# tanhuajie/Pytorch-RT1-for-Distributed-Training

Measured on AMD Instinct MI355X. Metric: train samples/sec (whole node), RT-1 Language-Table, 1/2/4/8 MI355X, higher is better.
Workload: dtype bf16; 1 GPU; model=RT-1 (FiLM-EfficientNet-B3 + TokenLearner-8 + 8-layer transformer, 35.3M params), global_batch=128, batch_per_gpu=128, seq_len=6, parallelism=dp1, backend=hip, hipgraph=True, step=graph, graph_segments=1, tuned_library_gemms=True, full=False

## Files before the change

pytorch_rt1_for_distributed_training_amd/csrc/bindings.cpp:

```cpp
#include <algorithm>
#include <cmath>
#include <cstdlib>

#include <torch/extension.h>
#include <c10/hip/HIPStream.h>
#include <hip/hip_runtime.h>

#include "rt1_kernels.h"

namespace {

hipStream_t cur_stream() { return c10::hip::getCurrentHIPStream().stream(); }

bool sync_check() {
    static const bool on = [] {
        const char* e = std::getenv("RT1_SYNC_CHECK");
        return e != nullptr && *e != '\0' && *e != '0';
    }();
    return on;
}

void check_launch(int err, const char* what) {
    TORCH_CHECK(err == 0, what, ": HIP launch failed: ", hipGetErrorString((hipError_t)err));
    if (sync_check()) {
// ... 777 lines not shown
    } else {
        check_launch(rt1_dw_bwd_fused(bp(dA), y2p, gate.data_ptr<float>(), rb.data_ptr<float>(), sc2.data_ptr<float>(),
                                      sh2.data_ptr<float>(), mu2.data_ptr<float>(), rs2.data_ptr<float>(),
                                      g2.data_ptr<float>(), mdz2.data_ptr<float>(), mdzx2.data_ptr<float>(),
                                      w.data_ptr<float>(), nullptr, nullptr, sc1.data_ptr<float>(), sh1.data_ptr<float>(),
                                      1, mu1.data_ptr<float>(), rs1.data_ptr<float>(), N, H, W, C, (int)k, gx, bp(dx),
                                      pa.data_ptr<float>(), pb.data_ptr<float>(), part.data_ptr<float>(), cur_stream(), 1,
                                      zout ? 1 : 0, bp(x), bp(we), cin),
                     "dw_bwd_fused_x");
    }
    return {dx, sum0(part).view({C, k * k}), pa, pb};
}

std::vector<at::Tensor> gemm(at::Tensor A, at::Tensor B, bool nn, OptT bias, OptT scale, OptT shift, OptT gate,
                             int64_t hw, bool out_f32, bool stats, int64_t cfg, bool store_a) {
    check_bf(A, "A"); check_bf(B, "B");
    TORCH_CHECK(A.dim() == 2 && B.dim() == 2, "gemm: 2-D operands");
    const int64_t M = A.size(0), K = A.size(1);
    const int64_t N = nn ? B.size(1) : B.size(0);
    TORCH_CHECK((nn ? B.size(0) : B.size(1)) == K, "gemm: inner dimensions differ");
    TORCH_CHECK(M > 0 && N % 8 == 0 && K % 8 == 0 && N > 0 && K > 0, "gemm: N and K must be multiples of 8");
    TORCH_CHECK(M < ((int64_t)1 << 31) && N * K < ((int64_t)1 << 31), "gemm: too large");
    TORCH_CHECK(reinterpret_cast<uintptr_t>(A.data_ptr()) % 16 == 0 && reinterpret_cast<uintptr_t>(B.data_ptr()) % 16 == 0,
                "gemm: operands must be 16-byte aligned");
    check_opt_f(bias, "bias", N);
    const bool pro = scale.has_value() && scale->defined();
    if (pro) {
        check_f(*scale, "scale", K); check_f(*shift, "shift", K);
        TORCH_CHECK(hw > 0 && M % hw == 0, "gemm: hw must divide M");
        check_f(*gate, "gate", (M / hw) * K);
        TORCH_CHECK(!out_f32, "gemm: the prologue path writes bf16");
    }
    TORCH_CHECK(!(stats && out_f32), "gemm: statistics describe a bf16 output");
    TORCH_CHECK(!store_a || pro, "gemm: store_a stores the prologue's rebuilt operand");
    auto C = at::empty({M, N}, A.options().dtype(out_f32 ? at::kFloat : at::kBFloat16));
    at::Tensor aout;
    if (store_a) aout = at::empty_like(A);
    at::Tensor ps, pq;
    if (stats) {
        const int tm = rt1_gemm_tiles_m((int)M, (int)N, (int)K, (int)cfg);
        ps = at::empty({tm, N}, f32(A));
        pq = at::empty({tm, N}, f32(A));
    }
    check_launch(rt1_gemm(bp(A), bp(B), C.data_ptr(), (int)M, (int)N, (int)K, nn ? 1 : 0, fpo(bias), fpo(scale),
                          fpo(shift), fpo(gate), (int)hw, out_f32 ? 1 : 0, stats ? ps.data_ptr<float>() : nullptr,
                          stats ? pq.data_ptr<float>() : nullptr, (int)cfg, store_a ? bp(aout) : nullptr,
                          cur_stream()), "gemm");
    std::vector<at::Tensor> out{C};
    if (stats) { out.push_back(ps); out.push_back(pq); }
    if (store_a) out.push_back(aout);
    return out;
}

at::Tensor film_fwd(at::Tensor xe, int64_t K, at::Tensor w, at::Tensor bias, at::Tensor cmap, int64_t total,
                    int64_t cfg) {
    check_bf(xe, "xe"); check_bf(w, "w");
    TORCH_CHECK(xe.dim() == 2 && w.dim() == 2 && w.size(1) == K && K <= xe.size(1), "film_fwd: xe [M, >= K], w [N, K]");
    const int64_t M = xe.size(0), N = w.size(0);
    TORCH_CHECK(M > 0 && N % 8 == 0 && K % 8 == 0 && xe.size(1) % 8 == 0, "film_fwd: N, K, lda multiples of 8");
    check_f(bias, "bias", N);
    TORCH_CHECK(cmap.is_cuda() && cmap.is_contiguous() && cmap.scalar_type() == at::kInt && cmap.numel() == N,
                "film_fwd: cmap must be an int32 [N / 4, 4] GPU tensor");
    TORCH_CHECK(total == M * N, "film_fwd: total must be M * N");
    auto out = at::empty({total}, f32(xe));
    check_launch(rt1_gemm_cmap(bp(xe), (int)xe.size(1), bp(w), out.data_ptr<float>(), (int)M, (int)N, (int)K,
                               bias.data_ptr<float>(), cmap.data_ptr<int>(), (int)cfg, cur_stream()), "film_fwd");
    return out;
}

std::vector<at::Tensor> film_wgrad(at::Tensor dflat, at::Tensor cmap, at::Tensor xe, int64_t K, int64_t splits,
                                   int64_t tile) {
    check_bf(xe, "xe");
    TORCH_CHECK(xe.dim() == 2 && K <= xe.size(1), "film_wgrad: xe [M, >= K]");
    const int64_t M = xe.size(0), N = cmap.numel();
    check_f(dflat, "dflat", M * N);
    TORCH_CHECK(cmap.is_cuda() && cmap.is_contiguous() && cmap.scalar_type() == at::kInt && N % 8 == 0 && K % 8 == 0,
                "film_wgrad: cmap int32 [N / 4, 4], N and K multiples of 8");
    auto a = xe.size(1) == K ? xe : xe.narrow(1, 0, K).contiguous();
    const int s = (int)std::max<int64_t>(1, std::min<int64_t>(splits, (M + 63) / 64));
    auto part = at::empty({s, N, K}, f32(xe));
    auto dbp = at::empty({s, N}, f32(xe));
    check_launch(rt1_wgrad_dymap(dflat.data_ptr<float>(), cmap.data_ptr<int>(), bp(a), M, (int)N, (int)K, s,
                                 part.data_ptr<float>(), dbp.data_ptr<float>(), (int)tile, cur_stream()),
                 "film_wgrad");
    if (s == 1) return {part[0], dbp[0]};
    return {sum0(part), sum0(dbp)};
}

std::vector<at::Tensor> gemm256(at::Tensor A, at::Tensor B, bool nn, OptT bias, OptT scale, OptT shift, OptT gate,
                                int64_t hw, bool stats, bool store_a, int64_t bn) {
    check_bf(A, "A"); check_bf(B, "B");
    TORCH_CHECK(A.dim() == 2 && B.dim() == 2, "gemm256: 2-D operands");
    const int64_t M = A.size(0), K = A.size(1);
    const int64_t N = nn ? B.size(1) : B.size(0);
    TORCH_CHECK((nn ? B.size(0) : B.size(1)) == K, "gemm256: inner dimensions differ");
    TORCH_CHECK(M > 0 && N > 0 && K > 0 && N % 8 == 0 && K % 8 == 0, "gemm256: N and K must be multiples of 8");
    TORCH_CHECK(M < ((int64_t)1 << 31) && M * K < ((int64_t)1 << 40), "gemm256: too large");
    TORCH_CHECK(reinterpret_cast<uintptr_t>(A.data_ptr()) % 16 == 0 && reinterpret_cast<uintptr_t>(B.data_ptr()) % 16 == 0,
                "gemm256: operands must be 16-byte aligned");
    TORCH_CHECK(bn == 128 || bn == 256, "gemm256: bn must be 128 or 256");
    check_opt_f(bias, "bias", N);
    const bool pro = scale.has_value() && scale->defined();
    if (pro) {
        TORCH_CHECK(!nn, "gemm256: the operand prologue is an NT path");
        check_f(*scale, "scale", K); check_f(*shift, "shift", K);
        TORCH_CHECK(hw > 0 && M % hw == 0, "gemm256: hw must divide M");
// ... 570 lines not shown
                           ln ? rs.data_ptr<float>() : nullptr, cur_stream()), "resid");
    if (ln) return {out, xn, mu, rs};
    return {out};
}

std::vector<at::Tensor> tf_drop_bwd(at::Tensor dout, double p, int64_t seed, OptT seed_dev) {
    check_rows512(dout, "dout", at::kFloat);
    const int T = (int)dout.size(0);
    const int grid = rt1_tf_grid(T);
    auto dh = at::empty({T, 512}, dout.options().dtype(at::kBFloat16));
    auto part = at::empty({grid, 512}, dout.options());
    check_launch(rt1_drop_bwd(dout.data_ptr<float>(), T, (float)p, (uint32_t)seed, seed_ptr(seed_dev), bp(dh),
                              part.data_ptr<float>(), grid,
                              cur_stream()), "drop_bwd");
    return {dh, sum0(part)};
}


namespace rt1comm {
void register_comm(py::module_& m);
}
namespace rt1head {
void register_head(py::module_& m);
}

PYBIND11_MODULE(_rt1_hip, m) {
    m.doc() = "RT-1 HIP/CDNA4 kernels (gfx950)";
    m.def("flat_adam", &flat_adam, "fused Adam/AdamW over flat fp32 buffers");
    m.def("flat_adam_dev", &flat_adam_dev, "fused Adam/AdamW, step/lr read from a device tensor (graph-replayable)");
    m.def("flat_adam_clip_dev", &flat_adam_clip_dev, "flat_adam_dev obeying clip_state (clip coefficient, skipped step)");
    m.def("flat_adam_ema_dev", &flat_adam_ema_dev, "flat_adam_dev / flat_adam_clip_dev that also updates the EMA of the weights");
    m.def("flat_adam_groups_dev", &flat_adam_groups_dev,
          "the device-state Adam forms (plain, clip, EMA, both) with lr / weight_decay per parameter group");
    m.def("gradnorm_partials", &gradnorm_partials, "fp64 partial sums grad_sumsq writes for n floats");
    m.def("grad_sumsq", &grad_sumsq, "deterministic sum of squares of a flat fp32 gradient -> fp64 partials");
    m.def("grad_clip_finalize", &grad_clip_finalize, "partials -> clip_state {norm, coef, ok, counters}");
    m.def("buffer_guard_", &buffer_guard_, "ok ? shadow = buf : buf = shadow");
    m.def("bn_stats", &bn_stats);
    m.def("bn_finalize", &bn_finalize);
    m.def("xgram", &xgram);
    m.def("gemm_tail", &gemm_tail, py::arg("A"), py::arg("B"), py::arg("A2"), py::arg("B2"), py::arg("bias") = py::none(),
          py::arg("res") = py::none(), py::arg("rmul") = py::none(), py::arg("rhw") = 1, py::arg("cfg") = -1);
    m.def("gemm256", &gemm256, py::arg("A"), py::arg("B"), py::arg("nn") = false, py::arg("bias") = py::none(),
          py::arg("scale") = py::none(), py::arg("shift") = py::none(), py::arg("gate") = py::none(),
          py::arg("hw") = 0, py::arg("stats") = false, py::arg("store_a") = false, py::arg("bn") = 256);
    m.def("film_fwd", &film_fwd, py::arg("xe"), py::arg("K"), py::arg("w"), py::arg("bias"), py::arg("cmap"),
          py::arg("total"), py::arg("cfg") = -1);
    m.def("film_wgrad", &film_wgrad, py::arg("dflat"), py::arg("cmap"), py::arg("xe"), py::arg("K"),
          py::arg("splits") = 1, py::arg("tile") = 0);
    m.def("gemm", &gemm, py::arg("A"), py::arg("B"), py::arg("nn") = false, py::arg("bias") = py::none(),
          py::arg("scale") = py::none(), py::arg("shift") = py::none(), py::arg("gate") = py::none(),
          py::arg("hw") = 0, py::arg("out_f32") = false, py::arg("stats") = false, py::arg("cfg") = -1,
          py::arg("store_a") = false);
    m.def("x_bn_stats", &x_bn_stats);
    m.def("bn_from_gram", &bn_from_gram);
    m.def("dw_x_supported", &dw_x_supported);
    m.def("dw_tile_info", &dw_tile_info);
    m.def("dw_fwd_x", &dw_fwd_x);
    m.def("dw_bwd_fused_x", &dw_bwd_fused_x, py::arg("dA"), py::arg("y2"), py::arg("gate"), py::arg("rb"),
          py::arg("sc2"), py::arg("sh2"), py::arg("mu2"), py::arg("rs2"), py::arg("g2"), py::arg("mdz2"),
          py::arg("mdzx2"), py::arg("w"), py::arg("k"), py::arg("x"), py::arg("we"), py::arg("sc1"), py::arg("sh1"),
          py::arg("mu1"), py::arg("rs1"), py::arg("max_blocks"), py::arg("zout") = true);
    m.def("bn_apply", &bn_apply);
    m.def("bn_bwd_reduce", &bn_bwd_reduce);
    m.def("bn_bwd_finalize", &bn_bwd_finalize);
    m.def("bn_bwd_finalize_new", &bn_bwd_finalize_new);
    m.def("bn_bwd_finalize_pw", &bn_bwd_finalize_pw);
    m.def("bn_bwd_apply", &bn_bwd_apply, py::arg("G"), py::arg("rs"), py::arg("rb"), py::arg("HW"), py::arg("y"),
          py::arg("scale"), py::arg("shift"), py::arg("mean"), py::arg("rstd"), py::arg("gamma"), py::arg("act"),
          py::arg("mdz"), py::arg("mdzx"), py::arg("keep") = py::none());
    m.def("dw_fwd", &dw_fwd);
    m.def("dw_bwd_data", &dw_bwd_data);
    m.def("dw_bwd_weight", &dw_bwd_weight);
    m.def("dw_bwd_fused", &dw_bwd_fused, py::arg("dA"), py::arg("y2"), py::arg("gate"), py::arg("rb"), py::arg("sc2"),
          py::arg("sh2"), py::arg("mu2"), py::arg("rs2"), py::arg("g2"), py::arg("mdz2"), py::arg("mdzx2"), py::arg("w"),
          py::arg("k"), py::arg("x1"), py::arg("sc1"), py::arg("sh1"), py::arg("act1"), py::arg("mu1"), py::arg("rs1"),
          py::arg("max_blocks"), py::arg("variant") = -1, py::arg("zout") = false, py::arg("res") = py::none(),
          py::arg("rmul") = py::none());
    m.def("gram", &gram, "{x^T x, sum_m x} fp32 of x [M, C] bf16 in one MFMA pass", py::arg("x"),
          py::arg("variant") = -1, py::arg("splits") = 0);
    m.def("wgrad", &wgrad, "1x1-conv weight gradient dy^T a on MFMA (optional BN/act/gate prologue on a)",
          py::arg("dy"), py::arg("a"), py::arg("scale") = py::none(), py::arg("shift") = py::none(),
          py::arg("gate") = py::none(), py::arg("act") = 0, py::arg("hw") = 0, py::arg("variant") = -1,
          py::arg("splits") = -1, py::arg("partials") = false, py::arg("sums") = false);
    m.def("crop_resize_u8", &crop_resize_u8, "Pillow-exact random-resized-crop of raw uint8 frames (GPU)");
    m.def("crop_resize_gather_u8", &crop_resize_gather_u8,
          "crop_resize_u8 over frames gathered by index from an HBM-resident [F, h, w, 3] table");
    m.def("multi_reduce_copy_", &multi_reduce_copy_, "dst[i] = fixed-order sum of splits[i] partials of src[i]",
          py::arg("dst"), py::arg("src"), py::arg("splits"), py::arg("sstride"));
    m.def("multi_copy_", &multi_copy_, "dst[i].copy_(src[i]) for many same-dtype tensors, 128 per launch");
    m.def("multi_reduce_add_", &multi_reduce_add_, "dst[i] += fixed-order sum of splits[i] partials of src[i]",
          py::arg("dst"), py::arg("src"), py::arg("splits"), py::arg("sstride"));
    m.def("multi_add_", &multi_add_, "dst[i] += src[i] for many fp32 tensors, 128 per launch");
    m.def("colsum", &colsum_py, "deterministic fixed-order sum over dim 0 (fp32/bf16 in, fp32 out)");
    m.def("frame_pool", &frame_pool);
    m.def("block_tail", &block_tail);
    m.def("tail_bwd_reduce", &tail_bwd_reduce);
    m.def("stem_fwd", &stem_fwd);
    m.def("stem_bwd_weight", &stem_bwd_weight, py::arg("img"), py::arg("shift"), py::arg("dy"), py::arg("max_blocks"),
          py::arg("bn_x") = py::none(), py::arg("scale") = py::none(), py::arg("shift_bn") = py::none(),
          py::arg("mean") = py::none(), py::arg("rstd") = py::none(), py::arg("gamma") = py::none(),
          py::arg("mdz") = py::none(), py::arg("mdzx") = py::none());
    m.def("attn_fwd", &attn_fwd, py::arg("qkv"), py::arg("L"), py::arg("Kimg"), py::arg("scale"), py::arg("drop_p"),
          py::arg("seed"), py::arg("seed_dev") = py::none());
    m.def("se_bn_bwd_reduce", &se_bn_bwd_reduce);
    m.def("proj_bwd", &proj_bwd, "project-conv backward sums + dWp from (dy3, y2) per frame (skinny blocks)");
// ... 30 lines not shown
```

pytorch_rt1_for_distributed_training_amd/csrc/kernels/gemm.hip:

```cpp
#include "common.h"

using namespace rt1;

namespace {

typedef short bf16x8 __attribute__((ext_vector_type(8)));
typedef short bf16x4 __attribute__((ext_vector_type(4)));
typedef float f32x4 __attribute__((ext_vector_type(4)));
typedef __attribute__((address_space(3))) bf16x4 lds_v4;

constexpr int BLOCK = 256;
constexpr int BK = 64;
constexpr int LDK = BK + 8;

__device__ __forceinline__ bf16x8 tr_read8(const bf16_t* base0, const bf16_t* base1) {
    const bf16x4 a = __builtin_amdgcn_ds_read_tr16_b64_v4i16((lds_v4*)base0);
    const bf16x4 b = __builtin_amdgcn_ds_read_tr16_b64_v4i16((lds_v4*)base1);
    return bf16x8{a[0], a[1], a[2], a[3], b[0], b[1], b[2], b[3]};
}

struct GemmArgs {
    const bf16_t* A;
    const bf16_t* B;
    void* C;
// ... 251 lines not shown
                u.x = pack2(v[0], v[1]);
                u.y = pack2(v[2], v[3]);
                *reinterpret_cast<uint2*>(reinterpret_cast<bf16_t*>(g.C) + m * N + n) = u;
                if constexpr (STATS) {
                    const float s0 = __uint_as_float(u.x << 16), s1 = __uint_as_float(u.x & 0xffff0000u);
                    const float s2 = __uint_as_float(u.y << 16), s3 = __uint_as_float(u.y & 0xffff0000u);
                    ssum[i][0] += s0; ssq[i][0] = fmaf(s0, s0, ssq[i][0]);
                    ssum[i][1] += s1; ssq[i][1] = fmaf(s1, s1, ssq[i][1]);
                    ssum[i][2] += s2; ssq[i][2] = fmaf(s2, s2, ssq[i][2]);
                    ssum[i][3] += s3; ssq[i][3] = fmaf(s3, s3, ssq[i][3]);
                }
            }
        }
    }
    if constexpr (STATS) {
#pragma unroll
        for (int i = 0; i < S::NT; ++i)
#pragma unroll
            for (int e = 0; e < 4; ++e) {
#pragma unroll
                for (int o = 1; o < 16; o <<= 1) {
                    ssum[i][e] += __shfl_xor(ssum[i][e], o, 64);
                    ssq[i][e] += __shfl_xor(ssq[i][e], o, 64);
                }
            }
        __syncthreads();
        float* red = reinterpret_cast<float*>(smem);
        if (lr == 0) {
#pragma unroll
            for (int i = 0; i < S::NT; ++i)
#pragma unroll
                for (int e = 0; e < 4; ++e) {
                    const int c = wn * S::WTN + i * 16 + lh * 4 + e;
                    red[(wm * 2) * BN + c] = ssum[i][e];
                    red[(wm * 2 + 1) * BN + c] = ssq[i][e];
                }
        }
        __syncthreads();
        for (int c = t; c < BN; c += BLOCK) {
            float a = 0.f, q = 0.f;
#pragma unroll
            for (int w = 0; w < WM; ++w) {
                a += red[(w * 2) * BN + c];
                q += red[(w * 2 + 1) * BN + c];
            }
            if (n0 + c < N) {
                g.ps[(int64_t)tm * N + n0 + c] = a;
                g.pq[(int64_t)tm * N + n0 + c] = q;
            }
        }
    }
}

struct Cfg { int bm, bn; };
constexpr Cfg CFGS[] = {{128, 128}, {64, 256}, {256, 64}, {64, 64}, {128, 64}};
constexpr int NCFG = 5;

int pick_cfg(int M, int N, int K, int cfg) {
    if (cfg >= 0 && cfg < NCFG) return cfg;
    (void)K;
    if (N <= 64) return 2;
    if (M <= 16384 && N >= 1024) return 1;
    return 0;
}

template <int BM, int BN, int WM, bool NN>
int launch_cfg(const GemmArgs& a, bool pro, bool f32, bool stats, hipStream_t st) {
    using S = GShape<BM, BN, WM, NN>;
    static_assert(BM * (BN + 8) * 2 <= S::lds, "LDS-staged store tile fits");
    const int tiles = ((a.M + BM - 1) / BM) * ((a.N + BN - 1) / BN);
    const dim3 grid(tiles);
    if constexpr (!NN) {
        if (a.A2) {
            if (pro || f32 || stats) return (int)hipErrorInvalidValue;
            hipLaunchKernelGGL((gemm_kernel<BM, BN, WM, false, false, false, false, true>), grid, dim3(BLOCK), S::lds,
                               st, a);
            return (int)hipGetLastError();
        }
    } else {
        if (a.A2) return (int)hipErrorInvalidValue;
    }
    static_assert(WM * 2 * BN * 4 <= S::lds, "stats scratch fits");
#define G(P, F, ST) hipLaunchKernelGGL((gemm_kernel<BM, BN, WM, NN, P, F, ST>), grid, dim3(BLOCK), S::lds, st, a)
    if (pro) {
        if (f32) return (int)hipErrorInvalidValue;
        if (stats) G(true, false, true); else G(true, false, false);
    } else if (f32) {
        if (stats) return (int)hipErrorInvalidValue;
        G(false, true, false);
    } else {
        if (stats) G(false, false, true); else G(false, false, false);
    }
#undef G
    return (int)hipGetLastError();
}

template <bool NN>
int launch_any(int cfg, const GemmArgs& a, bool pro, bool f32, bool stats, hipStream_t st) {
    switch (cfg) {
        case 0: return launch_cfg<128, 128, 2, NN>(a, pro, f32, stats, st);
        case 1: return launch_cfg<64, 256, 1, NN>(a, pro, f32, stats, st);
        case 2: return launch_cfg<256, 64, 4, NN>(a, pro, f32, stats, st);
        case 3: return launch_cfg<64, 64, 2, NN>(a, pro, f32, stats, st);
        default: return launch_cfg<128, 64, 2, NN>(a, pro, f32, stats, st);
    }
}

}

extern "C" {

int rt1_gemm_tiles_m(int M, int N, int K, int cfg) {
    const Cfg c = CFGS[pick_cfg(M, N, K, cfg)];
    return (M + c.bm - 1) / c.bm;
}

int rt1_gemm(const bf16_t* A, const bf16_t* B, void* C, int M, int N, int K, int nn, const float* bias,
             const float* scale, const float* shift, const float* gate, int hw, int out_f32, float* ps, float* pq,
             int cfg, bf16_t* aout, hipStream_t st) {
    if (M <= 0 || N <= 0 || K <= 0 || (N % 8) || (K % 8)) return (int)hipErrorInvalidValue;
    const bool pro = scale != nullptr;
    if (pro && (!shift || !gate || hw <= 0 || M % hw)) return (int)hipErrorInvalidValue;
    if ((ps != nullptr) != (pq != nullptr) || (aout && !pro)) return (int)hipErrorInvalidValue;
    GemmArgs a{A, B, C, M, N, K, bias, scale, shift, gate, hw, ps, pq, aout, nullptr, nullptr, 0, nullptr, nullptr, 1, K,
               nullptr};
    const bool stats = ps != nullptr;
    const int c = pick_cfg(M, N, K, cfg);
    return nn ? launch_any<true>(c, a, pro, out_f32, stats, st) : launch_any<false>(c, a, pro, out_f32, stats, st);
}

int rt1_gemm_tail(const bf16_t* A, const bf16_t* B, int M, int N, int K, const bf16_t* A2, const bf16_t* B2, int K2,
                  const float* bias, const bf16_t* res, const float* rmul, int rhw, bf16_t* C, int cfg,
                  hipStream_t st) {
    if (M <= 0 || N <= 0 || K <= 0 || K2 <= 0 || (N % 8) || (K % 8) || (K2 % 8) || !A2 || !B2)
        return (int)hipErrorInvalidValue;
    if (res && (!rmul || rhw <= 0 || M % rhw)) return (int)hipErrorInvalidValue;
    GemmArgs a{A, B, C, M, N, K, bias, nullptr, nullptr, nullptr, 1, nullptr, nullptr, nullptr, A2, B2, K2, res, rmul,
               rhw > 0 ? rhw : 1, K, nullptr};
    return launch_any<false>(pick_cfg(M, N, K, cfg), a, false, false, false, st);
}

int rt1_gemm_cmap(const bf16_t* A, int lda, const bf16_t* B, float* C, int M, int N, int K, const float* bias,
                  const int* cmap, int cfg, hipStream_t st) {
    if (M <= 0 || N <= 0 || K <= 0 || (N % 8) || (K % 8) || lda < K || (lda % 8) || !cmap)
        return (int)hipErrorInvalidValue;
    GemmArgs a{A, B, C, M, N, K, bias, nullptr, nullptr, nullptr, 1, nullptr, nullptr, nullptr, nullptr, nullptr, 0,
               nullptr, nullptr, 1, lda, reinterpret_cast<const int4*>(cmap)};
    return launch_any<false>(pick_cfg(M, N, K, cfg), a, false, true, false, st);
}

}
```

pytorch_rt1_for_distributed_training_amd/csrc/rt1_kernels.h:

```cpp
#pragma once
#include <hip/hip_runtime.h>
#include <stdint.h>

extern "C" {

int rt1_flat_adam(float* p, const float* g, float* m, float* v, int64_t n, float lr, float beta1, float beta2,
                  float eps, float weight_decay, float step_size, float inv_sqrt_bc2, float grad_scale,
                  hipStream_t stream);
int rt1_flat_adam_dev(float* p, const float* g, float* m, float* v, int64_t n, const float* state, float beta1,
                      float beta2, float eps, float weight_decay, float grad_scale, hipStream_t stream);
int rt1_flat_adam_clip_dev(float* p, const float* g, float* m, float* v, int64_t n, const float* state,
                           const float* clip_state, float beta1, float beta2, float eps, float weight_decay,
                           float grad_scale, hipStream_t stream);
int rt1_flat_adam_ema_dev(float* p, const float* g, float* m, float* v, float* ema, int64_t n, const float* state,
                          const float* clip_state, float* ema_state, float beta1, float beta2, float eps,
                          float weight_decay, float grad_scale, float one_minus_decay, int warmup,
                          hipStream_t stream);
int rt1_flat_adam_groups_dev(float* p, const float* g, float* m, float* v, float* ema, int64_t n, const float* state,
                             const float* group_state, const uint8_t* chunk_group, int G, const float* clip_state,
                             float* ema_state, float beta1, float beta2, float eps, float grad_scale,
                             float one_minus_decay, int warmup, hipStream_t stream);

int rt1_gradnorm_partials(int64_t n);
int rt1_grad_sumsq(const float* g, int64_t n, double* partials, hipStream_t stream);
// ... 21 lines not shown
                               hipStream_t st);
int rt1_bn_bwd_finalize(const float* pdz, const float* pdzx, int P, int C, double count, float* dgamma, float* dbeta,
                        float* mdz, float* mdzx, hipStream_t st, int accumulate);
int rt1_bn_bwd_apply(const rt1_bf16* G, const float* rs, const float* rb, int64_t HW, const rt1_bf16* y, int64_t M,
                     int C, const float* scale, const float* shift, const float* mean, const float* rstd,
                     const float* gamma, int act, const float* mdz, const float* mdzx, rt1_bf16* dy, hipStream_t st,
                     const float* keep = nullptr);

int rt1_dw_grid(int N, int H, int W, int C, int k, int s, int max_blocks_x, int pro, int epi);
int rt1_dw_wgrad_grid(int N, int H, int W, int C, int k, int s, int max_blocks_x, int pro);
int rt1_dw_bwd_grid(int N, int H, int W, int C, int k, int s, int max_blocks_x, int epi);
int rt1_dw_fwd(const rt1_bf16* x, const float* w, const float* scale, const float* shift, int act, int N, int H, int W,
               int C, int k, int s, int grid_x, rt1_bf16* out, float* psum, float* psq, hipStream_t st);
int rt1_dw_bwd_data(const rt1_bf16* dy, const float* w, const float* wflip, int N, int H, int W, int C, int k, int s,
                    int grid_x,
                    rt1_bf16* dx, const rt1_bf16* y_in, const float* scale, const float* shift, const float* mean,
                    const float* rstd, float* pdz, float* pdzx, hipStream_t st);
int rt1_dw_bwd_weight(const rt1_bf16* dy, const rt1_bf16* x, const float* scale, const float* shift, int act, int N,
                      int H, int W, int C, int k, int s, int grid_x, float* dwp, hipStream_t st);
int rt1_dw_bwd_uses_uni(int variant, int pro, int epi);
int rt1_dw_bwd_fused_s2_grid(int N, int H, int W, int C, int k, int max_blocks_x, int epi, int cin);
int rt1_dw_bwd_fused_s2(const rt1_bf16* dA, const rt1_bf16* y2, const float* gate, const float* rb,
                        const float* scale2, const float* shift2, const float* mean2, const float* rstd2,
                        const float* gamma2, const float* mdz2, const float* mdzx2, const float* w,
                        const rt1_bf16* x1, const float* scale1, const float* shift1, const float* mean1,
                        const float* rstd1, int N, int H, int W, int C, int k, int grid_x, rt1_bf16* dx, float* pdz,
                        float* pdzx, float* dwp, hipStream_t st, int zout, const rt1_bf16* xin,
                        const rt1_bf16* we, int cin);
int rt1_dw_bwd_fused_grid(int N, int H, int W, int C, int k, int max_blocks_x, int pro, int epi, int variant,
                          int cin);
int rt1_dw_bwd_fused(const rt1_bf16* dA, const rt1_bf16* y2, const float* gate, const float* rb, const float* scale2,
                     const float* shift2, const float* mean2, const float* rstd2, const float* gamma2,
                     const float* mdz2, const float* mdzx2, const float* w, const float* wflip, const rt1_bf16* x1,
                     const float* scale1,
                     const float* shift1, int act1, const float* mean1, const float* rstd1, int N, int H, int W, int C,
                     int k, int grid_x, rt1_bf16* dx, float* pdz, float* pdzx, float* dwp, hipStream_t st,
                     int variant, int zout, const rt1_bf16* xin, const rt1_bf16* we, int cin,
                     const rt1_bf16* res = nullptr, const float* rmul = nullptr);
int rt1_dw_x_supported(int cin, int C, int k, int s);
int rt1_dw_grid_x(int N, int H, int W, int C, int k, int s, int cin, int max_blocks_x);
int rt1_dw_tile_info(int which, int H, int W, int C, int k, int s, int cin, int* out);
int rt1_dw_fwd_x(const rt1_bf16* x, int cin, const rt1_bf16* we, const float* w, const float* scale1,
                 const float* shift1, int N, int H, int W, int C, int k, int s, int grid_x, rt1_bf16* out, float* psum,
                 float* psq, hipStream_t st);
int rt1_gemm_tiles_m(int M, int N, int K, int cfg);
int rt1_gemm_cmap(const rt1_bf16* A, int lda, const rt1_bf16* B, float* C, int M, int N, int K, const float* bias,
                  const int* cmap, int cfg, hipStream_t st);
int rt1_gemm(const rt1_bf16* A, const rt1_bf16* B, void* C, int M, int N, int K, int nn, const float* bias,
             const float* scale, const float* shift, const float* gate, int hw, int out_f32, float* ps, float* pq,
             int cfg, rt1_bf16* aout, hipStream_t st);
int rt1_gemm_tail(const rt1_bf16* A, const rt1_bf16* B, int M, int N, int K, const rt1_bf16* A2, const rt1_bf16* B2,
                  int K2, const float* bias, const rt1_bf16* res, const float* rmul, int rhw, rt1_bf16* C, int cfg,
                  hipStream_t st);
int rt1_g256_tiles_m(int M);
int rt1_g256(const rt1_bf16* A, const rt1_bf16* B, rt1_bf16* C, int M, int N, int K, int nn, const float* bias,
             const float* scale, const float* shift, const float* gate, int hw, rt1_bf16* aout, float* ps, float* pq,
             int bn, hipStream_t st);
int rt1_xgram_grid(int64_t M, int cin);
int rt1_xgram(const rt1_bf16* x, int64_t M, int cin, int grid, float* work, double* out, hipStream_t st);
int rt1_bn_from_gram(const double* G, const double* sx, const rt1_bf16* we, int cin, int C, double count,
                     const float* gamma, const float* beta, float eps, float momentum, float* running_mean,
                     float* running_var, float* scale, float* shift, float* save_mean, float* save_rstd,
                     hipStream_t st);
int rt1_bn_from_wg(const float* WG, const float* sx, const rt1_bf16* we, int cin, int C, double count,
                         const float* gamma, const float* beta, float eps, float momentum, float* running_mean,
                         float* running_var, float* scale, float* shift, float* save_mean, float* save_rstd,
                         hipStream_t st);

int rt1_frame_splits(int N, int HW, int C);
int rt1_frame_pool(const rt1_bf16* y, const rt1_bf16* G, int N, int HW, int C, const float* scale, const float* shift,
                   int act, int splits, float* pool, hipStream_t st);
int rt1_se_bn_bwd_reduce(const rt1_bf16* G, const rt1_bf16* y, int N, int HW, int C, const float* scale,
                         const float* shift, const float* mean, const float* rstd, int splits, float* out,
                         hipStream_t st);
int rt1_block_tail(const rt1_bf16* y3, int64_t M, int HW, int C, const float* scale, const float* shift,
                   const float* keep, const rt1_bf16* skip, const float* fmul, const float* fadd, rt1_bf16* out,
                   hipStream_t st);
int rt1_tail_bwd_reduce(const rt1_bf16* dout, const rt1_bf16* y3, int N, int HW, int C, const float* scale,
                        const float* shift, const float* mean, const float* rstd, const float* keep,
                        const rt1_bf16* skip, const float* fmul, int splits, float* dmul, float* dadd, float* pdz,
                        float* pdzx, hipStream_t st);

int rt1_stem_grid(int N, int H, int W, int max_blocks);
int rt1_stem_fwd(const void* img, int img_is_u8, const int* shift, const float* w, int N, int H, int W, int Cout,
                 int grid, rt1_bf16* out, float* psum, float* psq, hipStream_t st);
int rt1_stem_bwd_weight(const void* img, int img_is_u8, const int* shift, const rt1_bf16* dy, int N, int H, int W,
                        int Cout, int grid, float* dwp, hipStream_t st, const rt1_bf16* bn_x = nullptr,
                        const float* bn_scale = nullptr, const float* bn_shift = nullptr,
                        const float* bn_mean = nullptr, const float* bn_rstd = nullptr,
                        const float* bn_gamma = nullptr, const float* bn_mdz = nullptr,
                        const float* bn_mdzx = nullptr);

int rt1_attn_fwd(const rt1_bf16* qkv, rt1_bf16* out, float* lse, int B, int S, int H, int L, int Kimg, float scale,
                 float drop_p, uint32_t seed, const uint32_t* seed_dev, hipStream_t st);
int rt1_attn_keepmask(uint8_t* keep, int BH, int S, float drop_p, uint32_t seed, const uint32_t* seed_dev,
                      hipStream_t st);
int rt1_attn_bwd(const rt1_bf16* qkv, const rt1_bf16* out, const rt1_bf16* dout, const float* lse, rt1_bf16* dqkv,
                 int B, int S, int H, int L, int Kimg, float scale, float drop_p, uint32_t seed,
                 const uint32_t* seed_dev, hipStream_t st);

int rt1_attn_bwd_long(const rt1_bf16* qkv, const rt1_bf16* out, const rt1_bf16* dout, const float* lse,
                      rt1_bf16* dqkv, int B, int S, int H, int L, int Kimg, float scale, float drop_p, uint32_t seed,
                      const uint32_t* seed_dev, hipStream_t st);

int rt1_action_tokenize(const void* const* comps, const int* kind, const int* dim, int n, const float* low,
                        const float* high, int rows, int V, int64_t* out64, int* out32, hipStream_t st);
// ... 115 lines not shown
```

pytorch_rt1_for_distributed_training_amd/ops/backbone.py:

```python
from __future__ import annotations

import functools
import os
from dataclasses import dataclass, fields
from typing import List, Optional

import torch
import torch.nn.functional as F

from . import switches
from ._ext import load
from ..parallel.flat import defer_partials

ACT_NONE, ACT_SILU = 0, 1
MAX_BLOCKS = 2048
BF = torch.bfloat16


def _ext():
    return load()


def _mm(a: torch.Tensor, b: torch.Tensor) -> torch.Tensor:
    return torch.mm(a, b)


PW_BLOCKS = 2048


def _pw_blocks(M: int) -> int:
    return 512 if 500_000 <= M <= 2_000_000 else PW_BLOCKS


_DW_BWD_BLOCKS = {(38, 288): 1024, (38, 192): 512, (19, 288): 512, (19, 576): 256}
STEM_FWD_BLOCKS, STEM_BWD_BLOCKS, XMODE_BLOCKS = 3072, 1536, 4096
_TIMING = os.environ.get("RT1_BLOCK_TIMING", "0") == "1"
TIMING_EVENTS: List = []


def _mark(name: str):
    if _TIMING:
        ev = torch.cuda.Event(enable_timing=True)
        ev.record()
        TIMING_EVENTS.append((name, ev))


_GEMM_PROJ_TILE = {(1392, 232): 1, (816, 232): 1}
_GEMM_PROJ_DGRAD_TILE = {(1392, 232): 0, (816, 232): 0}
_Z_GEMM_TILE = {(1392, 232): -1, (2304, 384): -1}


@dataclass(frozen=True)
class RouteFlags:
    pw_tall: bool
    g256: bool
    wgrad_mfma: bool
    gram_sx: bool
    dw_fused: bool
    dw_s2_fused: bool
    dw_variant: int
    dw_res: bool
    pw_pro: bool
    proj_bwd: bool
    se_fused: bool
    stem_in_block0: bool
    stem_bn_bwd: bool
    pw_bwd_z: bool
    pw_z_wide: bool
    z_gemm: str
    xmode: str
    gram_bn: bool
    gemm_proj: bool
    gemm_proj_dgrad: bool
    tall_res: bool

    @classmethod
    def from_switches(cls, get=switches.get) -> "RouteFlags":
        cast = {"bool": lambda v: v != "0", "int": int, "str": str}
        return cls(**{f.name: cast[f.type](get(f.name)) for f in fields(cls)})

    g256_stats = property(lambda f: {(384, 1536), (384, 2304)} if f.g256 else set())
    gemm_proj_cfg = property(lambda f: _GEMM_PROJ_TILE if f.gemm_proj else {})
    gemm_proj_dgrad_cfg = property(lambda f: _GEMM_PROJ_DGRAD_TILE if f.gemm_proj_dgrad else {})
    z_gemm_cfg = property(lambda f: {"0": {}, "2": _Z_GEMM_TILE}.get(f.z_gemm, {(1392, 232): -1}))
    xmode_shapes = property(lambda f: {"0": set(), "all": None}.get(f.xmode, {(24, 144, 3, 2)}))


FLAGS = RouteFlags.from_switches()
_SHADOW = None


def set_weight_shadow(views):
    global _SHADOW
    _SHADOW = views


def _bf(w: torch.Tensor) -> torch.Tensor:
    if _SHADOW is not None:
        s = _SHADOW.get(w.data_ptr())
        if s is not None and s.shape == w.shape:
            return s
    return w.to(BF)


def _lin(a: torch.Tensor, w: torch.Tensor) -> torch.Tensor:
    ext = _ext()
    if ext.pw_gemm_supported(a.shape[1], w.shape[0]):
        return ext.pw_gemm(a, w.contiguous(), _pw_blocks(a.shape[0]))[0]
    if FLAGS.pw_tall and a.shape[0] >= 4096 and ext.pw_tall_preferred(a.shape[1], w.shape[0]):
        return ext.pw_tall(a.contiguous(), w.contiguous())[0]
    return torch.mm(a, w.t())


def _lin_bn(a: torch.Tensor, w: torch.Tensor, bnc: "BNCtx", training: bool, pro=None):
    ext = _ext()
    if pro is not None:
        sc, sh, gate, hw, store = pro
        res = ext.pw_gemm(a, w.contiguous(), _pw_blocks(a.shape[0]), training, sc, sh, gate, hw, store)
        consts = bnc.train_consts(res[1], res[2], a.shape[0]) if training else bnc.eval_consts()
        return res[0], consts, (res[-1] if store else None)
    if training and ext.pw_stats_supported(a.shape[1], w.shape[0]):
        y, ps, pq = ext.pw_gemm(a, w.contiguous(), _pw_blocks(a.shape[0]), True)
        return y, bnc.train_consts(ps, pq, a.shape[0])
    if training and (a.shape[1], w.shape[0]) in FLAGS.g256_stats:
        y, ps, pq = ext.gemm256(a, w.contiguous(), False, stats=True, bn=256)
        return y, bnc.train_consts(ps, pq, a.shape[0])
    y = _lin(a, w)
    return y, _bn_train_or_eval(bnc, training, y)


def _pw_bwd_blocks(M: int, z: bool = False) -> int:
    if M >= 10_000_000:
        return 4096
    if M >= 3_000_000:
        return 3072 if z else 2048
    return 512


def _dw_wgrad_blocks(C: int) -> int:
    return 4096 if C <= 144 else 2048


def _mm_f32(a: torch.Tensor, b: torch.Tensor) -> torch.Tensor:
    try:
        return torch.mm(a, b, out_dtype=torch.float32)
    except (TypeError, RuntimeError):
        return torch.mm(a, b).float()


def _wgrad_splits(M: int, out_elems: int) -> int:
    if M >= 8_000_000:
        S = 256
    elif M >= 2_000_000:
        S = 128
    elif M >= 600_000:
        S = 256
    elif M >= 150_000:
        S = 64 if out_elems < 40_000 else 32
    elif M >= 16_384:
# ... 750 lines not shown
```

pytorch_rt1_for_distributed_training_amd/ops/switches.py:

```python
from __future__ import annotations

import os
from typing import Dict

DEFAULTS: Dict[str, str] = {
    "pw_tall": "1",
    "g256": "1",
    "wgrad_mfma": "1",
    "wgrad_deep": "1",
    "dw_fused": "1",
    "dw_s2_fused": "1",
    "dw_variant": "1",
    "dw_res": "1",
    "pw_pro": "1",
    "proj_bwd": "1",
    "se_fused": "1",
    "stem_in_block0": "1",
    "stem_bn_bwd": "1",
    "pw_bwd_z": "1",
    "pw_z_wide": "1",
    "z_gemm": "1",
    "xmode": "1",
    "gram_bn": "1",
    "gemm_proj": "1",
    "gemm_proj_dgrad": "1",
    "tall_res": "1",
    "gram_sx": "1",
    "tf_wgrad": "1",
    "tf_gemm": "1",
    "tf_fuse_ln": "1",
    "multi_copy": "1",
}


def _parse(spec: str) -> Dict[str, str]:
    out: Dict[str, str] = {}
    for item in filter(None, (s.strip() for s in spec.split(","))):
        name, sep, value = item.partition("=")
        name = name.strip()
        if not sep or name not in DEFAULTS:
            raise ValueError(f"RT1_AB: unknown or malformed switch {item!r}; known: {', '.join(sorted(DEFAULTS))}")
        out[name] = value.strip()
    return out


_OVERRIDES = _parse(os.environ.get("RT1_AB", ""))


def get(name: str) -> str:
    if name not in DEFAULTS:
        raise KeyError(name)
    return _OVERRIDES.get(name, DEFAULTS[name])


def on(name: str) -> bool:
    return get(name) != "0"


def overrides() -> Dict[str, str]:
    return dict(_OVERRIDES)
```

Measured before the change: 1433 samples/s.

## Add row-resident GEMM kernel for K=232 to N=1392 pointwise expansion

Adds a new bf16 GEMM kernel that keeps each workgroup's 128-row A tile resident in registers for the full K (up to 256) and streams B in 64-column tiles through double-buffered LDS. The epilogue for the previous tile is overlapped with the MFMA loop of the current one via a per-wave LDS patch, producing coalesced stores. It is routed only for the (K=232, N=1392) forward linear, replacing the pw_gemm/tall path, to cut repeated A reloads and improve overlap. It costs high register pressure and only covers the small-K case.

```diff
diff --git a/pytorch_rt1_for_distributed_training_amd/csrc/bindings.cpp b/pytorch_rt1_for_distributed_training_amd/csrc/bindings.cpp
--- a/pytorch_rt1_for_distributed_training_amd/csrc/bindings.cpp
+++ b/pytorch_rt1_for_distributed_training_amd/csrc/bindings.cpp
@@ -853,6 +853,20 @@
     return out;
 }
 
+bool gemm_rows_supported(int64_t K) { return rt1_gemm_rows_supported((int)K) != 0; }
+at::Tensor gemm_rows(at::Tensor A, at::Tensor B) {
+    check_bf(A, "A"); check_bf(B, "B");
+    TORCH_CHECK(A.dim() == 2 && B.dim() == 2 && A.size(1) == B.size(1), "gemm_rows: A [M, K], B [N, K]");
+    const int64_t M = A.size(0), K = A.size(1), N = B.size(0);
+    TORCH_CHECK(M > 0 && N > 0 && N % 8 == 0 && gemm_rows_supported(K), "gemm_rows: no kernel for K=", K, " N=", N);
+    TORCH_CHECK(M < ((int64_t)1 << 31) && N * K < ((int64_t)1 << 31), "gemm_rows: too large");
+    TORCH_CHECK(reinterpret_cast<uintptr_t>(A.data_ptr()) % 16 == 0 && reinterpret_cast<uintptr_t>(B.data_ptr()) % 16 == 0,
+                "gemm_rows: operands must be 16-byte aligned");
+    auto C = at::empty({M, N}, A.options());
+    check_launch(rt1_gemm_rows(bp(A), bp(B), bp(C), (int)M, (int)N, (int)K, cur_stream()), "gemm_rows");
+    return C;
+}
+
 at::Tensor film_fwd(at::Tensor xe, int64_t K, at::Tensor w, at::Tensor bias, at::Tensor cmap, int64_t total,
                     int64_t cfg) {
     check_bf(xe, "xe"); check_bf(w, "w");
@@ -1529,6 +1543,8 @@
           py::arg("scale") = py::none(), py::arg("shift") = py::none(), py::arg("gate") = py::none(),
           py::arg("hw") = 0, py::arg("out_f32") = false, py::arg("stats") = false, py::arg("cfg") = -1,
           py::arg("store_a") = false);
+    m.def("gemm_rows_supported", &gemm_rows_supported);
+    m.def("gemm_rows", &gemm_rows, py::arg("A"), py::arg("B"));
     m.def("x_bn_stats", &x_bn_stats);
     m.def("bn_from_gram", &bn_from_gram);
     m.def("dw_x_supported", &dw_x_supported);
diff --git a/pytorch_rt1_for_distributed_training_amd/csrc/kernels/gemm.hip b/pytorch_rt1_for_distributed_training_amd/csrc/kernels/gemm.hip
--- a/pytorch_rt1_for_distributed_training_amd/csrc/kernels/gemm.hip
+++ b/pytorch_rt1_for_distributed_training_amd/csrc/kernels/gemm.hip
@@ -327,6 +327,145 @@
     }
 }
 
+constexpr int R_BM = 128, R_BN = 64, R_KP = 256, R_KS = R_KP / 32;
+constexpr int R_LDK = R_KP + 8;
+constexpr int R_LDN = R_BN + 8;
+constexpr int R_PB = 8;
+constexpr int R_PATCH = 16 * R_LDN;
+
+constexpr int R_B_ELEMS = R_BN * R_LDK;
+constexpr size_t R_LDS = (size_t)(2 * R_B_ELEMS + 4 * R_PATCH) * 2;
+static_assert(2 * R_LDS <= 160 * 1024, "two workgroups per CU");
+
+__device__ __forceinline__ void lds_only_barrier() {
+    asm volatile("s_waitcnt lgkmcnt(0)" ::: "memory");
+    __builtin_amdgcn_s_barrier();
+    asm volatile("" ::: "memory");
+}
+
+__global__ __launch_bounds__(BLOCK, 2) void gemm_rows_kernel(const bf16_t* __restrict__ A, const bf16_t* __restrict__ B,
+                                                             bf16_t* __restrict__ C, int M, int N, int K) {
+    extern __shared__ __attribute__((aligned(16))) char smem[];
+    const int t = threadIdx.x, lane = t & 63, wave = t >> 6;
+    const int lr = lane & 15, lh = lane >> 4;
+    constexpr int b_elems = R_B_ELEMS;
+    bf16_t* Bbuf = reinterpret_cast<bf16_t*>(smem);
+    bf16_t* patch = Bbuf + 2 * b_elems + wave * R_PATCH;
+    const int64_t m0 = (int64_t)blockIdx.x * R_BM + wave * 32;
+
+    bf16x8 fa[2][R_KS];
+#pragma unroll
+    for (int j = 0; j < 2; ++j)
+#pragma unroll
+        for (int ks = 0; ks < R_KS; ++ks) {
+            const int64_t m = m0 + j * 16 + lr;
+            const int k = ks * 32 + lh * 8;
+            uint4 u = make_uint4(0, 0, 0, 0);
+            if (m < M && k < K) u = *reinterpret_cast<const uint4*>(A + m * K + k);
+            fa[j][ks] = *reinterpret_cast<const bf16x8*>(&u);
+        }
+
+    uint4 rb[R_PB];
+    auto issue = [&](int s) {
+        const int n0 = s * R_BN;
+#pragma unroll
+        for (int i = 0; i < R_PB; ++i) {
+            const int v = t + i * BLOCK;
+            rb[i] = make_uint4(0, 0, 0, 0);
+            const int r = v >> 5, k = (v & 31) * 8;
+            if (n0 + r < N && k < K) rb[i] = *reinterpret_cast<const uint4*>(B + (int64_t)(n0 + r) * K + k);
+        }
+    };
+    auto stage = [&](int bsel) {
+        bf16_t* Bl = Bbuf + bsel * b_elems;
+#pragma unroll
+        for (int i = 0; i < R_PB; ++i) {
+            const int v = t + i * BLOCK;
+            const int r = v >> 5, k = (v & 31) * 8;
+            *reinterpret_cast<uint4*>(Bl + r * R_LDK + k) = rb[i];
+        }
+    };
+
+    const int steps = (N + R_BN - 1) / R_BN;
+    uint2 pk[2][4];
+    uint4 o0, o1, o2, o3;
+    int pn0 = 0;
+    const int pr = lane >> 3, pc = (lane & 7) * 8;
+    auto epi_lds = [&](int j, const uint2 (&q)[2][4], uint4& r0, uint4& r1) {
+#pragma unroll
+        for (int i = 0; i < 4; ++i) *reinterpret_cast<uint2*>(patch + lr * R_LDN + i * 16 + lh * 4) = q[j][i];
+        asm volatile("" ::: "memory");
+        r0 = *reinterpret_cast<const uint4*>(patch + pr * R_LDN + pc);
+        r1 = *reinterpret_cast<const uint4*>(patch + (pr + 8) * R_LDN + pc);
+        asm volatile("" ::: "memory");
+    };
+    auto epi_store = [&](int n0) {
+        if (n0 + pc < N) {
+            bf16_t* cp = C + (m0 + pr) * N + n0 + pc;
+            const int64_t left = M - (m0 + pr);
+            if (left > 0) *reinterpret_cast<uint4*>(cp) = o0;
+            if (left > 8) *reinterpret_cast<uint4*>(cp + 8 * (int64_t)N) = o1;
+            if (left > 16) *reinterpret_cast<uint4*>(cp + 16 * (int64_t)N) = o2;
+            if (left > 24) *reinterpret_cast<uint4*>(cp + 24 * (int64_t)N) = o3;
+        }
+    };
+    issue(0);
+    stage(0);
+    lds_only_barrier();
+    for (int s = 0; s < steps; ++s) {
+        if (s + 1 < steps) issue(s + 1);
+        const bf16_t* Bl = Bbuf + (s & 1) * b_elems;
+        f32x4 acc[4][2];
+#pragma unroll
+        for (int i = 0; i < 4; ++i)
+#pragma unroll
+            for (int j = 0; j < 2; ++j) acc[i][j] = f32x4{0.f, 0.f, 0.f, 0.f};
+        auto frags = [&](int ks, bf16x8 (&fb)[4]) {
+#pragma unroll
+            for (int i = 0; i < 4; ++i)
+                fb[i] = *reinterpret_cast<const bf16x8*>(Bl + (i * 16 + lr) * R_LDK + ks * 32 + lh * 8);
+        };
+        bf16x8 fb[2][4];
+        frags(0, fb[0]);
+#pragma unroll
+        for (int ks = 0; ks < R_KS; ++ks) {
+            if (ks + 1 < R_KS) frags(ks + 1, fb[(ks + 1) & 1]);
+            if (s > 0) {
+                if (ks == 0) epi_lds(0, pk, o0, o1);
+                if (ks == 1) epi_lds(1, pk, o2, o3);
+                if (ks == 3) epi_store(pn0);
+            }
+            __builtin_amdgcn_sched_barrier(0);
+#pragma unroll
+            for (int i = 0; i < 4; ++i)
+#pragma unroll
+                for (int j = 0; j < 2; ++j)
+                    acc[i][j] = __builtin_amdgcn_mfma_f32_16x16x32_bf16(fb[ks & 1][i], fa[j][ks], acc[i][j], 0, 0, 0);
+        }
+#pragma unroll
+        for (int j = 0; j < 2; ++j)
+#pragma unroll
+            for (int i = 0; i < 4; ++i) {
+                pk[j][i].x = pack2(acc[i][j][0], acc[i][j][1]);
+                pk[j][i].y = pack2(acc[i][j][2], acc[i][j][3]);
+            }
+        pn0 = s * R_BN;
+        if (s + 1 < steps) stage((s + 1) & 1);
+        lds_only_barrier();
+    }
+    epi_lds(0, pk, o0, o1);
+    epi_lds(1, pk, o2, o3);
+    epi_store(pn0);
+}
+
+int launch_rows(const bf16_t* A, const bf16_t* B, bf16_t* C, int M, int N, int K, hipStream_t st) {
+    static const hipError_t attr = hipFuncSetAttribute((const void*)gemm_rows_kernel,
+                                                       hipFuncAttributeMaxDynamicSharedMemorySize, (int)R_LDS);
+    if (attr != hipSuccess) return (int)attr;
+    hipLaunchKernelGGL(gemm_rows_kernel, dim3((M + R_BM - 1) / R_BM), dim3(BLOCK), R_LDS, st, A, B, C, M, N, K);
+    return (int)hipGetLastError();
+}
+
 struct Cfg { int bm, bn; };
 constexpr Cfg CFGS[] = {{128, 128}, {64, 256}, {256, 64}, {64, 64}, {128, 64}};
 constexpr int NCFG = 5;
@@ -415,6 +554,12 @@
     return launch_any<false>(pick_cfg(M, N, K, cfg), a, false, false, false, st);
 }
 
+int rt1_gemm_rows_supported(int K) { return K > 0 && K % 8 == 0 && K <= R_KP; }
+int rt1_gemm_rows(const bf16_t* A, const bf16_t* B, bf16_t* C, int M, int N, int K, hipStream_t st) {
+    if (M <= 0 || N <= 0 || (N % 8) || !rt1_gemm_rows_supported(K)) return (int)hipErrorInvalidValue;
+    return launch_rows(A, B, C, M, N, K, st);
+}
+
 int rt1_gemm_cmap(const bf16_t* A, int lda, const bf16_t* B, float* C, int M, int N, int K, const float* bias,
                   const int* cmap, int cfg, hipStream_t st) {
     if (M <= 0 || N <= 0 || K <= 0 || (N % 8) || (K % 8) || lda < K || (lda % 8) || !cmap)
diff --git a/pytorch_rt1_for_distributed_training_amd/csrc/rt1_kernels.h b/pytorch_rt1_for_distributed_training_amd/csrc/rt1_kernels.h
--- a/pytorch_rt1_for_distributed_training_amd/csrc/rt1_kernels.h
+++ b/pytorch_rt1_for_distributed_training_amd/csrc/rt1_kernels.h
@@ -97,6 +97,8 @@
 int rt1_gemm_tail(const rt1_bf16* A, const rt1_bf16* B, int M, int N, int K, const rt1_bf16* A2, const rt1_bf16* B2,
                   int K2, const float* bias, const rt1_bf16* res, const float* rmul, int rhw, rt1_bf16* C, int cfg,
                   hipStream_t st);
+int rt1_gemm_rows_supported(int K);
+int rt1_gemm_rows(const rt1_bf16* A, const rt1_bf16* B, rt1_bf16* C, int M, int N, int K, hipStream_t st);
 int rt1_g256_tiles_m(int M);
 int rt1_g256(const rt1_bf16* A, const rt1_bf16* B, rt1_bf16* C, int M, int N, int K, int nn, const float* bias,
              const float* scale, const float* shift, const float* gate, int hw, rt1_bf16* aout, float* ps, float* pq,
diff --git a/pytorch_rt1_for_distributed_training_amd/ops/backbone.py b/pytorch_rt1_for_distributed_training_amd/ops/backbone.py
--- a/pytorch_rt1_for_distributed_training_amd/ops/backbone.py
+++ b/pytorch_rt1_for_distributed_training_amd/ops/backbone.py
@@ -48,6 +48,7 @@
 _GEMM_PROJ_TILE = {(1392, 232): 1, (816, 232): 1}
 _GEMM_PROJ_DGRAD_TILE = {(1392, 232): 0, (816, 232): 0}
 _Z_GEMM_TILE = {(1392, 232): -1, (2304, 384): -1}
+_ROWS_FWD = {(232, 1392)} if switches.on("rows_fwd") else set()
 
 
 @dataclass(frozen=True)
@@ -105,6 +106,8 @@
 
 def _lin(a: torch.Tensor, w: torch.Tensor) -> torch.Tensor:
     ext = _ext()
+    if (a.shape[1], w.shape[0]) in _ROWS_FWD:
+        return ext.gemm_rows(a.contiguous(), w.contiguous())
     if ext.pw_gemm_supported(a.shape[1], w.shape[0]):
         return ext.pw_gemm(a, w.contiguous(), _pw_blocks(a.shape[0]))[0]
     if FLAGS.pw_tall and a.shape[0] >= 4096 and ext.pw_tall_preferred(a.shape[1], w.shape[0]):
diff --git a/pytorch_rt1_for_distributed_training_amd/ops/switches.py b/pytorch_rt1_for_distributed_training_amd/ops/switches.py
--- a/pytorch_rt1_for_distributed_training_amd/ops/switches.py
+++ b/pytorch_rt1_for_distributed_training_amd/ops/switches.py
@@ -24,6 +24,7 @@
     "gram_bn": "1",
     "gemm_proj": "1",
     "gemm_proj_dgrad": "1",
+    "rows_fwd": "1",
     "tall_res": "1",
     "gram_sx": "1",
     "tf_wgrad": "1",
```

After: 1433 samples/s, median of 4. No clear change (-0.0%).
